# mushroonhead/spatial-intention-maps

Measured on AMD Instinct MI355X. Metric: agent-state-stacks/sec (96×96×C maps) at 1/2/4/8 MI355X; HBM GB/s vs peak, higher is better.
Workload: dtype f32

## Files before the change

spatial-intention-maps_amd/csrc/get_state_body.inc:

```
    __shared__ __attribute__((aligned(16))) char smem[LDS_BYTES];
    Shared &sh = *reinterpret_cast<Shared *>(smem);
    float *dist = reinterpret_cast<float *>(smem + OFF_DIST);
    SsspScratch &S = *reinterpret_cast<SsspScratch *>(smem + OFF_UNION);
    float *tile = reinterpret_cast<float *>(smem + OFF_UNION);

    const int n = blockIdx.x;
    const int tid = threadIdx.x;
    const int H = cfg.H, W = cfg.W;
    if (tid == 0) STAMP_NB(77);
    simaps_agent ag = agents[n];
    const int nsrc = (cfg.use_shortest_path_to_receptacle_map ? 1 : 0) + (cfg.use_shortest_path_map ? 1 : 0);
    const int cs_waves = nsrc > 0 ? 4 * nsrc : (dbg.cspace ? 4 : 0);
    const bool early_tile =
        nsrc > 0 && (cfg.room_h + 2) * sssp_pitch(cfg.room_w) * 4 <= DIST_FLOATS * 4 - CMAP_BYTES;
    uint8_t *cmap = reinterpret_cast<uint8_t *>(smem) + (early_tile ? OFF_UNION - CMAP_BYTES : OFF_CMAP);
    const bool tail_cells = early_tile && !cfg.use_distance_to_receptacle_map &&
                            tail_cells_off(cfg.room_h, cfg.room_w) + LW * LW * 2 <= DIST_FLOATS * 4;
    if (tid < 16) (&sh.bar[0][0])[tid] = 0u;
    if (tid == 16) sh.scratch_free = cs_waves == 0;
#if defined(GS_SPEC) && !GS_MIXED
    OccLoad4<512> pre8;
    OccLoad4<256> pre4;
    const bool pre_occ = (tid >> 6) < cs_waves && nsrc > 0 && occ4_ok(H, W, cfg.room_j0);
    if (pre_occ) {
        const uint8_t *occ_slot = occupancy + (size_t)ag.map_slot * H * W;
        if (cs_waves == 8) cspace_load4<512>(pre8, occ_slot, H, W, cfg.room_i0, cfg.room_j0, cfg.room_h, tid);
        else cspace_load4<256>(pre4, occ_slot, H, W, cfg.room_i0, cfg.room_j0, cfg.room_h, tid);
    }
#endif
#ifdef GS_CACHED
    char *const sc_rec = (unsigned)ag.map_slot < (unsigned)cache_records
                             ? cache + (size_t)ag.map_slot * simaps_state_cache::record_bytes(GS_ROOM_H, GS_ROOM_W)
                             : nullptr;
    CachePre sc_pre;
    if (pre_occ) cache_preload<GS_ROOM_H, GS_ROOM_W>(sc_pre, sc_rec, tid);
    bool sc_join = false;
#endif
    simaps_env ev = envs[ag.env];
    int nr_cap = SIMAPS_MAX_ROBOTS;
    if (cfg.use_intention_channels)
        nr_cap = (C - 1 - !!cfg.use_robot_map - !!cfg.use_distance_to_receptacle_map -
                  !!cfg.use_shortest_path_to_receptacle_map - !!cfg.use_shortest_path_map - !!cfg.use_history_map -
                  !!cfg.use_intention_map) / (cfg.intention_channel_spatial ? 1 : 2) + 1;
    const bool bad_desc = (unsigned)(ev.num_robots - 1) >= (unsigned)SIMAPS_MAX_ROBOTS ||
                          (unsigned)ag.robot >= (unsigned)ev.num_robots ||
                          (cfg.use_intention_channels && ev.num_robots != nr_cap);
    ev.num_robots = min(max(ev.num_robots, 1), min(nr_cap, SIMAPS_MAX_ROBOTS));
    if ((unsigned)ag.robot >= (unsigned)ev.num_robots) ag.robot = 0;
    lds_barrier();
    if (tid == 0 && bad_desc) sh.bar[0][3] = 1u;
    if (tid == 0) STAMP_NB(0);
#if GS_MIXED && defined(SIMAPS_STATE16)
    uint16_t *out = state + (size_t)out_off[n];
#elif GS_MIXED
    float *out = state + (size_t)out_off[n];
#elif defined(GS_INTO)
    auto *out = state + (size_t)into_row * LW * LW * C;
#elif defined(SIMAPS_STATE16)
    uint16_t *out = state + (size_t)n * LW * LW * C;
#else
    float *out = state + (size_t)n * LW * LW * C;
#endif
    const RenderCtx rc{cfg, sh, out, C, n};
    if ((tid >> 6) < cs_waves) {
        const Group g{tid, 64 * cs_waves, sh.bar[0], cs_waves};
#if GS_MIXED
        const uint8_t *occ_base = occupancy + ((int64_t)map_off[ag.map_slot] - (int64_t)ag.map_slot * H * W);
        if (cs_waves == 8) sweep_track<512>(sh, S, dist, cfg, geo, ag, ev, robots, occ_base, nsrc, dbg, n, g, early_tile);
        else sweep_track<256>(sh, S, dist, cfg, geo, ag, ev, robots, occ_base, nsrc, dbg, n, g, early_tile);
#elif defined(GS_CACHED)
        sc_join = sweep_track_cached<GS_ROOM_H, GS_ROOM_W>(sh, S, dist, cfg, geo, ag, ev, robots, sc_rec, pre8, sc_pre, g);
#elif defined(GS_SPEC)
        if (cs_waves == 8)
            sweep_track<512, GS_ROOM_H, GS_ROOM_W>(sh, S, dist, cfg, geo, ag, ev, robots, occupancy, nsrc, dbg, n, g,
                                                   early_tile, &pre8);
        else
            sweep_track<256, GS_ROOM_H, GS_ROOM_W>(sh, S, dist, cfg, geo, ag, ev, robots, occupancy, nsrc, dbg, n, g,
                                                   early_tile, &pre4);
#else
        if (cs_waves == 8) sweep_track<512>(sh, S, dist, cfg, geo, ag, ev, robots, occupancy, nsrc, dbg, n, g, early_tile);
        else sweep_track<256>(sh, S, dist, cfg, geo, ag, ev, robots, occupancy, nsrc, dbg, n, g, early_tile);
#endif
#ifdef GS_CACHED
        if (!sc_join) STAMP_NB(7);
    }
    if ((tid >> 6) >= cs_waves || sc_join) {
        int nw = NT / 64 - cs_waves;
        Group g{tid - 64 * cs_waves, 64 * nw, sh.bar[1], nw};
        int t = sc_join ? SC_NO_PARAM_THREAD : g.t;
#else
        STAMP_NB(7);
    } else {
        const int nw = NT / 64 - cs_waves;
        const Group g{tid - 64 * cs_waves, 64 * nw, cs_waves ? sh.bar[1] : nullptr, nw};
        const int t = g.t;
#endif
        const simaps_robot *rb = robots + ev.robot_off;
        if (t == 0) {
            sh.nr = ev.num_robots;
            sh.me = ag.robot;
            sh.env = ag.env;
            sh.has_rec = ev.has_receptacle;
        }
        if (t == 64) {
            const simaps_robot &me = rb[ag.robot];
            sh.rot = rot_params(CROP, 90.0 - me.heading * RAD_TO_DEG, cfg.rotate_rounding == SIMAPS_ROT_PLAIN);
            pos_to_pix(me.x, me.y, H, W, sh.pi, sh.pj);
            STAMP_NB(72);
        }
        if (t >= 128 && t < 128 + ev.num_robots) {
            const int k = t - 128;
            const simaps_robot &r = rb[k];
            RobotP &P = sh.rob[k];
            if ((cfg.use_intention_map && r.intention_len > SIMAPS_MAX_PATH) ||
                (cfg.use_history_map && r.history_len > SIMAPS_MAX_PATH))
                __hip_atomic_store(&sh.bar[0][3], 1u, __ATOMIC_RELAXED, __HIP_MEMORY_SCOPE_WORKGROUP);
            robot_params(P, r, cfg, geo, H, W);
            if (k == 0) STAMP_NB(73);
        }
        {
            const int w8 = t >> 6;
            const bool z8 = g.n == 512;
            const int zt = z8 ? (w8 == 3 || w8 == 4 ? t - 192 : (w8 >= 6 ? t - 256 : -1)) : t;
            const int zn = z8 ? 256 : g.n;
            if (zt >= 0) {
                uint4 *cz = reinterpret_cast<uint4 *>(cmap);
                for (int k = zt; k < CMAP_BYTES / 16; k += zn) cz[k] = uint4{0u, 0u, 0u, 0u};
                if (early_tile) {
                    uint4 *tz = reinterpret_cast<uint4 *>(tile);
                    for (int k = SCRATCH_Q + zt; k < TILE * TILE / 4; k += zn) tz[k] = uint4{0u, 0u, 0u, 0u};
                }
            }
        }
        const bool segs = (cfg.use_history_map || cfg.use_intention_map) && t >= 320 &&
                          t < 320 + ev.num_robots * SEG_PER_ROBOT;
        if (segs) {
            seg_geom(sh, cfg, rb, paths, cfg.use_history_map ? 4 : cfg.intention_map_encoding, t - 320, ag.robot);
            if (t == 320) STAMP_NB(74);
        }
        if (t < 5 * 24) sh.mwin[t] = geo.mbits[t / 24][t % 24];
        if (t >= 192 && t < 192 + 20) {
            const int q = t - 192, m = q >> 2, f = q & 3;
            sh.mwin[120 + q] = f == 0 ? geo.mrow0[m] : f == 1 ? geo.mcol0[m] : f == 2 ? geo.mnrows[m] : geo.mncols[m];
        }
        if (t == 0) STAMP_NB(75);
#ifdef GS_CACHED
        if (sc_join || cache_verdict_hit(sh)) {
            nw = 12;
            g = Group{tid - 256, 768, sh.bar[1], 12};
        }
#endif
        g.sync();
        if (t == 0) STAMP_NB(9);
        if (segs) seg_ramp(sh, t - 320);
        if (cfg.use_intention_channels && t == 256) intention_channel_order(sh, cfg, rb);
#ifdef GS_CACHED
        t = g.t;
#endif

        if (t == 0) STAMP_NB(51);
        uint32_t *cmap32 = reinterpret_cast<uint32_t *>(cmap);
        const int ci0 = sh.pi - HALF_CROP, cj0 = sh.pj - HALF_CROP;
        const int ln = t & 63, wv = __builtin_amdgcn_readfirstlane(t >> 6);
        const int nrb = ev.num_robots, wpr = nrb <= nw ? nw / nrb : 1;
        for (int kk = wv; kk < nrb * wpr; kk += nw) {
            const int k = kk % nrb, sub = kk / nrb;
            const RobotP &P = sh.rob[k];
            const int bi0 = __builtin_amdgcn_readfirstlane(P.bi0), bi1 = __builtin_amdgcn_readfirstlane(P.bi1);
            const int bj0 = P.bj0, bj1 = P.bj1, st_i = P.st_i, st_j = P.st_j;
            const int type = P.type;
            const bool cube = type == SIMAPS_LIFTING && P.lifting;
            const unsigned code0 = P.code0;
            const Rot R{P.c, P.s, P.f0, P.f1, P.S0, P.S1};
            const int *mt = reinterpret_cast<const int *>(sh.mwin + 120 + 4 * type);
            const int *mc = reinterpret_cast<const int *>(sh.mwin + 120 + 4 * 4);
            const int mt0 = mt[0], mt1 = mt[1], mt2 = mt[2], mt3 = mt[3];
            const int mc0 = mc[0], mc1 = mc[1], mc2 = mc[2], mc3 = mc[3];
            for (int rp = sub; 2 * rp <= bi1 - bi0; rp += wpr) {
                const int gi = bi0 + 2 * rp + (ln >> 5), gj = bj0 + (ln & 31);
                unsigned code = 0;
                if (gi <= bi1 && gj <= bj1) {
                    int m0, m1;
                    const bool in = rot_src(R, LW, gi - st_i, gj - st_j, m0, m1);
                    if (in) {
                        const int r = m0 - mt0, cc = m1 - mt1;
                        if ((unsigned)r < (unsigned)mt2 && (unsigned)cc < (unsigned)mt3 && ((sh.mwin[type * 24 + r] >> cc) & 1u))
                            code = code0;
                        const int r2 = m0 - mc0, c2 = m1 - mc1;
                        if (cube && (unsigned)r2 < (unsigned)mc2 && (unsigned)c2 < (unsigned)mc3 && ((sh.mwin[4 * 24 + r2] >> c2) & 1u))
                            code |= 1u << 5;
                    }
                }
                const int ca = gi - ci0, cb = gj - cj0;
                if (code && (unsigned)ca < (unsigned)CROP && (unsigned)cb < (unsigned)CROP) {
                    const int pos = ca * CROP + cb;
                    atomicOr(&cmap32[pos >> 2], code << (8 * (pos & 3)));
                }
            }
        }
#ifdef GS_SPEC
        if (early_tile && cfg.use_shortest_path_to_receptacle_map && cfg.use_shortest_path_map)
            zero_scratch_early(sh, tile, g);
#endif
        g.sync();
        if (t == 0) STAMP_NB(1);
#if GS_MIXED
        const float *ovh = overhead + (size_t)map_off[ag.map_slot];
#else
        const float *ovh = overhead + (size_t)ag.map_slot * H * W;
#endif
        if (nw == 8) render_maps<18>(rc, g, geo, ovh, rb, paths, tile, cmap, early_tile, tail_cells, dist);
        else if (nw == 12) render_maps<12>(rc, g, geo, ovh, rb, paths, tile, cmap, early_tile, tail_cells, dist);
        else render_maps<9>(rc, g, geo, ovh, rb, paths, tile, cmap, early_tile, tail_cells, dist);
        if (t == 0) STAMP_NB(8);
    }
    lds_barrier();
    STAMP(4);

    STAMP(5);
    render_distance_channels(rc, ev, dist, nsrc, reinterpret_cast<const uint16_t *>(tile),
                             tail_cells ? reinterpret_cast<const uint16_t *>(reinterpret_cast<const char *>(dist) +
                                                                          tail_cells_off(cfg.room_h, cfg.room_w))
                                        : reinterpret_cast<const uint16_t *>(tile) + LW * LW);
    STAMP(6);

    if (nsrc > 0) {
        if (dbg.sources && tid < 2) {
            int32_t *o = dbg.sources + ((size_t)n * 2 + tid) * 4;
            const int s = sh.sp_slot[tid];
            if (s >= 0) { o[0] = sh.src_q[s][0]; o[1] = sh.src_q[s][1]; o[2] = sh.src_s[s][0]; o[3] = sh.src_s[s][1]; }
            else { o[0] = o[1] = o[2] = o[3] = -1; }
        }
    }
    if (tid == 0) {
        const unsigned f = group_faults(sh.bar, sh.rounds, nsrc);
#if defined(GS_INTO) && defined(GS_INTO_KID)
        post_faults(fault, f, GS_INTO_KID, n);
#elif defined(GS_INTO)
        post_faults(fault, f, SIMAPS_K_GET_STATE_INTO, n);
#else
        post_faults(fault, f, GS_MIXED ? SIMAPS_K_GET_STATE_MIXED : SIMAPS_K_GET_STATE, n);
#endif
        if (dbg.status) {
            int st = (f & SIMAPS_FAULT_ROUNDS ? 2 : 0) | (f & SIMAPS_FAULT_TIMEOUT ? 4 : 0) |
                     (f & SIMAPS_FAULT_DESCRIPTOR ? 8 : 0);
            for (int s = 0; s < nsrc; s++) st |= sh.src_ok[s] ? 0 : 1;
            dbg.status[n] = st | ((nsrc > 0 ? sh.rounds & 0xfffff : 0) << 8);
        }
    }
#ifdef SIMAPS_PHASE_STAMPS
    if (tid == 0 && blockIdx.x < MAX_STAMP_WG) g_stamps[blockIdx.x * NSTAMP + 10] = (unsigned long long)sh.rounds;
#endif
```

spatial-intention-maps_amd/csrc/simaps_spec_cached.hip:

```cpp
#define GS_SPEC
#define GS_CACHED
#define GS_ROOM_H RH
#define GS_ROOM_W RW
#define SIMAPS_DEVICE_ONLY
#include "simaps.hip"
#include "spec.h"
#include "state_cache.h"

namespace {
using namespace simaps_state_cache;
static_assert(WIN_PAD == RMAX && WIN_ROW_U32 * 4 == (int)sizeof(uint64_t) * WIN_WORDS, "the record's window rows are SsspScratch::win's");
static_assert(sizeof(B128) == 16, "a row of free bits");

constexpr int SC_NO_PARAM_THREAD = 1 << 20;
typedef unsigned u32x4 __attribute__((ext_vector_type(4)));

__device__ __forceinline__ unsigned &sc_diff(Shared &sh) { return sh.bar[3][0]; }
__device__ __forceinline__ unsigned &sc_verdict(Shared &sh) { return sh.bar[3][3]; }

struct CachePre {
    u32x4 key[4];
    uint32_t w[OccLoad4<512>::NQ], w2;
    u32x4 pf[5];
    uint32_t pft;
};
template <int RH, int RW>
struct HitSplit {
    static constexpr int cells = (RH + 2) * ((RW + 2) | 1);
    static constexpr int ROWS = (RH + 2 + 15) / 16, FULL = cells / 4 / 256, LAST = cells / 4 - 256 * FULL, TAIL = cells & 3;
    static_assert(ROWS <= 5 && FULL == 4, "CachePre::pf holds a thread's share");
};

template <int RH, int RW>
__device__ __forceinline__ void cache_preload(CachePre &P, const char *rec, int t)
{
    const __amdgpu_buffer_rsrc_t rs =
        __builtin_amdgcn_make_buffer_rsrc((void *)rec, (short)0, rec ? record_bytes(RH, RW) : 0, 0x00020000);
    const int lane = t & 63, wave = t >> 6;
    constexpr int whM = RH + 2 * RMAX;
#pragma unroll
    for (int k = 0; k < 4; k++) P.key[k] = __builtin_amdgcn_raw_buffer_load_b128(rs, 16 * k, 0, 0);
#pragma unroll
    for (int q = 0; q < OccLoad4<512>::NQ; q++) {
        const int rr = 2 * (wave + 8 * q) + (lane >> 5);
        P.w[q] = __builtin_amdgcn_raw_buffer_load_b32(rs, rr < whM ? OFF_WIN + (rr * WIN_ROW_U32 + ((lane >> 3) & 3)) * 4 : -1, 0, 0);
    }
    const int rr = t >> 2;
    P.w2 = __builtin_amdgcn_raw_buffer_load_b32(rs, rr < whM ? OFF_WIN + (rr * WIN_ROW_U32 + 4) * 4 : -1, 0, 0);
    using HS = HitSplit<RH, RW>;
    const bool rows = wave < 4;
    const int t2 = t - 256, arr = off_rec(RH) + REC_HDR;
#pragma unroll
    for (int k = 0; k < 5; k++) {
        const int r = (t >> 4) + 16 * k;
        const int o_row = k < HS::ROWS && r >= 1 && r <= RH ? off_free(RH) + (r - 1) * 16 : -1;
        const int o_arr = k < HS::FULL || t2 < HS::LAST ? arr + (t2 + 256 * k) * 16 : -1;
        P.pf[k] = __builtin_amdgcn_raw_buffer_load_b128(rs, rows ? o_row : o_arr, 0, 0);
    }
    P.pft = __builtin_amdgcn_raw_buffer_load_b32(rs, !rows && t2 < HS::TAIL ? arr + ((HS::cells & ~3) + t2) * 4 : -1, 0, 0);
}

__device__ __forceinline__ bool win_from_dwords_cmp(SsspScratch &S, const OccLoad4<512> &L, const CachePre &P, int whM, int t)
{
    static_assert(OccLoad4<512>::NU == 1, "one tail dword per thread");
    const int lane = t & 63, wave = t >> 6;
    uint32_t *win32 = reinterpret_cast<uint32_t *>(&S.win[0][0]);
    bool diff = false;
#pragma unroll
    for (int q = 0; q < OccLoad4<512>::NQ; q++) {
        unsigned x = nib4(L.v[q]) << (4 * (lane & 7));
        x |= (unsigned)__builtin_amdgcn_mov_dpp((int)x, 0x111, 0xf, 0xf, true);
        x |= (unsigned)__builtin_amdgcn_mov_dpp((int)x, 0x112, 0xf, 0xf, true);
        x |= (unsigned)__builtin_amdgcn_mov_dpp((int)x, 0x114, 0xf, 0xf, true);
        const int rr = 2 * (wave + 8 * q) + (lane >> 5);
        if ((lane & 7) == 7 && rr < whM) {
            win32[rr * 6 + ((lane >> 3) & 3)] = x;
            diff |= x != P.w[q];
        }
    }
    {
        const int rr = t >> 2;
        unsigned x = nib4(L.v2[0]) << (4 * (t & 3));
        x |= (unsigned)__builtin_amdgcn_mov_dpp((int)x, 0x111, 0xf, 0xf, true);
        x |= (unsigned)__builtin_amdgcn_mov_dpp((int)x, 0x112, 0xf, 0xf, true);
        if ((t & 3) == 3 && rr < whM) {
            win32[rr * 6 + 4] = x;
            diff |= x != P.w2;
        }
    }
    return diff;
}

__device__ __forceinline__ bool cache_verdict_hit(Shared &sh)
{
    unsigned v = 0;
    if ((threadIdx.x & 63) == 0) {
        unsigned spins = 0;
        while (!(v = __hip_atomic_load(&sc_verdict(sh), __ATOMIC_RELAXED, __HIP_MEMORY_SCOPE_WORKGROUP))) {
            __builtin_amdgcn_s_sleep(1);
            if (++spins > (1u << 22)) {
                __hip_atomic_store(&sh.bar[1][2], 1u, __ATOMIC_RELAXED, __HIP_MEMORY_SCOPE_WORKGROUP);
                break;
            }
        }
    }
    __builtin_amdgcn_fence(__ATOMIC_ACQUIRE, "workgroup", "local");
    return (unsigned)__builtin_amdgcn_readfirstlane((int)v) == 2u;
}

template <int RH, int RW>
__device__ __forceinline__ void sssp_rounds_swapped(Shared &sh, float *dist)
{
    const int wave = __builtin_amdgcn_readfirstlane((int)threadIdx.x >> 6);
    switch ((wave + 2 * ((wave >> 2) ^ 1)) & 3) {
    case 0: sssp_rounds_word<0, RH, RW, 1>(sh, dist); break;
    case 1: sssp_rounds_word<1, RH, RW, 1>(sh, dist); break;
    case 2: sssp_rounds_word<2, RH, RW, 1>(sh, dist); break;
    default: sssp_rounds_word<3, RH, RW, 1>(sh, dist); break;
    }
}

template <int RH, int RW>
__device__ __forceinline__ bool sweep_track_cached(Shared &sh, SsspScratch &S, float *dist, const simaps_config &cfg,
                                                   const Geometry &geo, const simaps_agent &ag, const simaps_env &ev,
                                                   const simaps_robot *__restrict__ robots, char *rec,
                                                   const OccLoad4<512> &occ4, const CachePre &P, const Group &g)
{
    constexpr int h = RH, w = RW, pw = (RW + 2) | 1, cells = (h + 2) * pw, whM = h + 2 * RMAX;
    static_assert(OFF_WIN + whM * WIN_ROW_U32 * 4 <= off_free(h) && off_rec(h) + REC_HDR + cells * 4 <= record_bytes(h, w),
                  "the record's parts");
    static_assert(REC_HDR == 16 && off_rec(h) % 16 == 0 && off_free(h) % 16 == 0, "16-byte aligned parts");
    const int t = g.t, H = cfg.H, W = cfg.W;
#ifdef SIMAPS_PHASE_STAMPS
    if (t == 0 && ag.map_slot >= 0) STAMP_NB(43);
#endif
    const simaps_robot *rb = robots + ev.robot_off;
    const int radius = geo.cspace_r[rb[ag.robot].type];
    int rq0 = 0, rq1 = 0;
    if (t == 0) {
        sh.h = h;
        sh.w = w;
        sh.i0 = cfg.room_i0;
        sh.j0 = cfg.room_j0;
        pos_to_pix(ev.receptacle_x, ev.receptacle_y, H, W, rq0, rq1);
        sh.src_q[0][0] = rq0;
        sh.src_q[0][1] = rq1;
        pos_to_pix(rb[ag.robot].x, rb[ag.robot].y, H, W, sh.src_q[1][0], sh.src_q[1][1]);
        sh.sp_slot[0] = 0;
        sh.sp_slot[1] = 1;
        sh.nsrc = 2;
    }
    const u32x4 key0 = {(unsigned)SIMAPS_STATE_CACHE_MAGIC, (unsigned)H, (unsigned)W, (unsigned)cfg.room_i0};
    const u32x4 key1 = {(unsigned)cfg.room_j0, (unsigned)h, (unsigned)w, (unsigned)radius};
    const u32x4 key2 = {(unsigned)ev.has_receptacle, (unsigned)rq0, (unsigned)rq1, 0u};
    bool diff = win_from_dwords_cmp(S, occ4, P, whM, t);
    if (t == 0) {
        const u32x4 d = (P.key[0] ^ key0) | (P.key[1] ^ key1) | (P.key[2] ^ key2);
        diff |= (d.x | d.y | d.z | d.w) != 0u;
    }
    if (__ballot(diff) && (t & 63) == 0)
        __hip_atomic_fetch_or(&sc_diff(sh), 1u, __ATOMIC_RELAXED, __HIP_MEMORY_SCOPE_WORKGROUP);
    g.sync();
    if (t == 0) STAMP_NB(15);
    const bool hit = __builtin_amdgcn_readfirstlane(
                         (int)__hip_atomic_load(&sc_diff(sh), __ATOMIC_RELAXED, __HIP_MEMORY_SCOPE_WORKGROUP)) == 0;
    if (t == 0) {
#ifdef SIMAPS_DIAG_VERDICT_LATE
        for (int k = 0; k < 8; k++) __builtin_amdgcn_s_sleep(127);
#endif
        __builtin_amdgcn_fence(__ATOMIC_RELEASE, "workgroup", "local");
        __hip_atomic_store(&sc_verdict(sh), hit ? 2u : 1u, __ATOMIC_RELAXED, __HIP_MEMORY_SCOPE_WORKGROUP);
    }
    const float scale = (float)cfg.shortest_path_map_scale;
    if (hit) {
        using HS = HitSplit<RH, RW>;
        static_assert(HS::cells == cells, "the same array");
        if (t >= 256) {
            const int t2 = t - 256;
            u32x4 *d4 = reinterpret_cast<u32x4 *>(dist);
#pragma unroll
            for (int k = 0; k < HS::FULL; k++) d4[t2 + 256 * k] = P.pf[k];
            if (t2 < HS::LAST) d4[t2 + 256 * HS::FULL] = P.pf[HS::FULL];
            if (t2 < HS::TAIL) reinterpret_cast<uint32_t *>(dist)[(cells & ~3) + t2] = P.pft;
            return true;
        }
        const Group g4{t, 256, sh.bar[0], 4};
        const int qr = sh.src_q[1][0] - cfg.room_i0, qc = sh.src_q[1][1] - cfg.room_j0;
        const bool q_in = (unsigned)qr < (unsigned)h && (unsigned)qc < (unsigned)w;
        auto publish = [&](bool fr) {
            sh.src_ok[1] = fr;
            sh.src_s[1][0] = sh.src_q[1][0];
            sh.src_s[1][1] = sh.src_q[1][1];
#pragma unroll
            for (int q = 0; q < 8; q++) {
                const int d2 = (q >> 1) & 3, word = q & 1, bit = fr ? (d2 < 2 ? qr : qc) : -1;
                sh.dirty[1][d2][word] = bit >= 0 && (bit >> 6) == word ? 1ull << (bit & 63) : 0ull;
            }
        };
        const int l16 = t & 15;
        float *D1 = dist + DIST_FLOATS;
        bool own = false, own_free = false;
#pragma unroll
        for (int k = 0; k < HS::ROWS; k++) {
            const int r = (t >> 4) + 16 * k;
            if (r < h + 2) {
                const B128 f = {P.pf[k].x | ((uint64_t)P.pf[k].y << 32), P.pf[k].z | ((uint64_t)P.pf[k].w << 32)};
                if (l16 == 0 && r >= 1 && r <= h) S.freeb[r - 1] = f;
                const bool qrow = q_in && r == qr + 1;
#pragma unroll
                for (int i = 0; i < (pw + 15) / 16; i++) {
                    const int c = l16 + 16 * i;
                    if (c < pw) {
                        const bool fc = c >= 1 && c <= w && b_test(f, c - 1);
                        const bool src = qrow && c == qc + 1;
                        own |= src;
                        own_free |= src && fc;
                        D1[r * pw + c] = src && fc ? 0.0f : (fc ? INFINITY : -INFINITY);
                    }
                }
            }
        }
        if (own || (t == 0 && !q_in)) publish(own_free);
        if (t == 0) {
            const u32x4 res = P.key[3];
            sh.src_s[0][0] = (int)res.x;
            sh.src_s[0][1] = (int)res.y;
            sh.src_ok[0] = (int)res.z;
            sh.dmax[0] = __uint_as_float(res.w);
            sh.unreach[0] = (__uint_as_float(res.w) / 96.0f) * scale;
            __hip_atomic_fetch_add(reinterpret_cast<unsigned *>(rec + offsetof(simaps_state_cache_header, hits)), 1u,
                                   __ATOMIC_RELAXED, __HIP_MEMORY_SCOPE_AGENT);
        }
        if (t < 6) (&sh.changed[0][0])[t] = 0;
        if (t == 6) sh.rounds = 0;
        g4.sync();
        if (t == 0) STAMP_NB(2);
        if (!sh.src_ok[1]) {
            if (t < 64)
                snap_wave(S.freeb, h, w, cfg.room_i0, cfg.room_j0, sh.src_q[1][0], sh.src_q[1][1], [&](int si, int sj) {
                    const int sr = si - cfg.room_i0, sc = sj - cfg.room_j0;
                    if (t == 0) {
                        sh.src_s[1][0] = si;
                        sh.src_s[1][1] = sj;
                        sh.src_ok[1] = 1;
                        D1[(sr + 1) * pw + sc + 1] = 0.0f;
                    }
                    if (t < 8) {
                        const int d2 = (t >> 1) & 3, word = t & 1, bit = d2 < 2 ? sr : sc;
                        sh.dirty[1][d2][word] = (bit >> 6) == word ? 1ull << (bit & 63) : 0ull;
                    }
                });
            g4.sync();
        }
        if (t == 0) {
            STAMP_NB(48);
            __builtin_amdgcn_fence(__ATOMIC_RELEASE, "workgroup", "local");
            __hip_atomic_store(&sh.scratch_free, 1, __ATOMIC_RELAXED, __HIP_MEMORY_SCOPE_WORKGROUP);
            STAMP_NB(3);
        }
        sssp_rounds_swapped<RH, RW>(sh, dist);
        const float m = max_finite_part(D1, cells, t, 256);
        if ((t & 63) == 0) sh.red[1][t >> 6] = m;
        g4.sync();
        if (t == 0) STAMP_NB(49);
        if (t == 1) {
            float mm = sh.red[1][0];
            for (int k = 1; k < 4; k++) mm = fmaxf(mm, sh.red[1][k]);
            sh.dmax[1] = mm;
            sh.unreach[1] = (mm / 96.0f) * scale;
        }
        if (t == 0) STAMP_NB(50);
        return false;
    }
    build_cspace<512>(S, nullptr, h, w, radius, g, dist, 2, &occ4, nullptr, H, W, cfg.room_i0, cfg.room_j0, true);
    if (t == 0) STAMP_NB(2);
    if (rec) {
        const uint32_t *win32 = reinterpret_cast<const uint32_t *>(&S.win[0][0]);
        uint32_t *rw = reinterpret_cast<uint32_t *>(rec + OFF_WIN);
        for (int k = t; k < whM * WIN_ROW_U32; k += 512)
            if (k % WIN_ROW_U32 != 5) rw[k] = win32[k];
        if (t < h) reinterpret_cast<B128 *>(rec + off_free(h))[t] = S.freeb[t];
    }
    snap_init_sources(sh, S, dist, 2, g);
    if (t == 0) {
        STAMP_NB(48);
        __builtin_amdgcn_fence(__ATOMIC_RELEASE, "workgroup", "local");
        __hip_atomic_store(&sh.scratch_free, 1, __ATOMIC_RELAXED, __HIP_MEMORY_SCOPE_WORKGROUP);
        STAMP_NB(3);
    }
    sssp_rounds_swapped<RH, RW>(sh, dist);
    {
        const int s = (t >> 8) ^ 1;
        if (rec && s == 0) rec_export(rec + off_rec(h), dist, h, w, sh.src_ok[0], nullptr, t & 255, 256);
        const float m = max_finite_part(dist + s * DIST_FLOATS, cells, t & 255, 256);
        if ((t & 63) == 0) sh.red[s][(t >> 6) & 3] = m;
    }
    g.sync();
    if (t == 0) STAMP_NB(49);
    sssp_max_final(sh, 2, 4, scale, t);
    if (rec && t == 0) {
        const bool good = sh.rounds < (1 << 20);
        u32x4 *hd = reinterpret_cast<u32x4 *>(rec);
        hd[0] = u32x4{good ? key0[0] : 0u, key0[1], key0[2], key0[3]};
        hd[1] = key1;
        hd[2] = key2;
        const bool ok0 = sh.src_ok[0] != 0;
        hd[3] = u32x4{ok0 ? (unsigned)sh.src_s[0][0] : ~0u, ok0 ? (unsigned)sh.src_s[0][1] : ~0u, ok0 ? 1u : 0u,
                      __float_as_uint(sh.dmax[0])};
        __hip_atomic_fetch_add(reinterpret_cast<unsigned *>(rec + offsetof(simaps_state_cache_header, misses)), 1u,
                               __ATOMIC_RELAXED, __HIP_MEMORY_SCOPE_AGENT);
    }
    if (t == 0) STAMP_NB(50);
    return false;
}

template <int MH, int MW, int RH, int RW>
__global__ void __launch_bounds__(NT) get_state_cached_kernel(
    simaps_config cfg_in, Geometry geo, const simaps_agent *__restrict__ agents, const simaps_env *__restrict__ envs,
    const simaps_robot *__restrict__ robots, const double *__restrict__ paths, const uint8_t *__restrict__ occupancy,
    const float *__restrict__ overhead, float *__restrict__ state, int C, unsigned *fault, char *cache, int cache_records)
{
    simaps_config cfg = cfg_in;
    cfg.use_robot_map = 1;
    cfg.use_distance_to_receptacle_map = 0;
    cfg.use_shortest_path_to_receptacle_map = 1;
    cfg.use_shortest_path_map = 1;
    cfg.use_intention_map = 1;
    cfg.use_history_map = 0;
    cfg.use_intention_channels = 0;
    cfg.layout_chw = 1;
    cfg.H = MH;
    cfg.W = MW;
    cfg.room_h = RH;
    cfg.room_w = RW;
    const simaps_debug dbg = {};
#define GS_MIXED 0
#include "get_state_body.inc"
#undef GS_MIXED
}
}

namespace simaps_state_cache {
void launch_get_state(const simaps_config &cfg, const simaps::Geometry &geo, int N, const simaps_agent *agents,
                      const simaps_env *envs, const simaps_robot *robots, const double *paths,
                      const uint8_t *occupancy, const float *overhead, float *state, int C, unsigned *fault,
                      void *cache, int cache_records, hipStream_t stream)
{
    constexpr int MH = SIMAPS_ROOM_SMALL_H, MW = SIMAPS_ROOM_SMALL_W, RH = SIMAPS_ROOM_SMALL_RH, RW = SIMAPS_ROOM_SMALL_RW;
    hipLaunchKernelGGL((get_state_cached_kernel<MH, MW, RH, RW>), dim3(N), dim3(NT), 0, stream, cfg, geo, agents, envs,
                       robots, paths, occupancy, overhead, state, C, fault, (char *)cache, cache_records);
}

#if defined(SIMAPS_PHASE_STAMPS) || defined(SIMAPS_LIGHT_STAMPS)
int read_stamps(unsigned long long *host_out)
{
    return hipMemcpyFromSymbol(host_out, HIP_SYMBOL(g_stamps), sizeof(g_stamps)) == hipSuccess ? 0 : SIMAPS_EHIP;
}
#endif
}
```

Baseline: 10.98 million.

## Load cached distance array straight into LDS with buffer-load DMA on hit

On a cache hit, the cached distance array is no longer preloaded into registers by the upper waves and then stored to LDS. It is fetched after the verdict using buffer_load ... lds, which writes directly into shared memory, and the wait is deferred until just before the map-rendering group sync. Preload loads are also restricted to the waves that use them (key only in wave 0, window rows only for in-range waves), which lowers register pressure and wasted VMEM issue. The trade-off is that the array fetch now starts only after the hit verdict rather than being prefetched, so its latency has to be hidden behind the cmap/render work. It also relies on hand-written inline asm that manipulates M0.

```diff
diff --git a/spatial-intention-maps_amd/csrc/get_state_body.inc b/spatial-intention-maps_amd/csrc/get_state_body.inc
--- a/spatial-intention-maps_amd/csrc/get_state_body.inc
+++ b/spatial-intention-maps_amd/csrc/get_state_body.inc
@@ -202,6 +202,9 @@
         if (early_tile && cfg.use_shortest_path_to_receptacle_map && cfg.use_shortest_path_map)
             zero_scratch_early(sh, tile, g);
 #endif
+#if defined(GS_CACHED) && !defined(SIMAPS_DIAG_ARRAY_LATE)
+        if (sc_join) sc_retire_array();
+#endif
         g.sync();
         if (t == 0) STAMP_NB(1);
 #if GS_MIXED
@@ -214,6 +217,12 @@
         else render_maps<9>(rc, g, geo, ovh, rb, paths, tile, cmap, early_tile, tail_cells, dist);
         if (t == 0) STAMP_NB(8);
     }
+#if defined(GS_CACHED) && defined(SIMAPS_DIAG_ARRAY_LATE)
+    if (sc_join) {
+        hit_array_dma<GS_ROOM_H, GS_ROOM_W>(dist, sc_rec, tid - 256);
+        sc_retire_array();
+    }
+#endif
     lds_barrier();
     STAMP(4);
 
diff --git a/spatial-intention-maps_amd/csrc/simaps_spec_cached.hip b/spatial-intention-maps_amd/csrc/simaps_spec_cached.hip
--- a/spatial-intention-maps_amd/csrc/simaps_spec_cached.hip
+++ b/spatial-intention-maps_amd/csrc/simaps_spec_cached.hip
@@ -21,44 +21,100 @@
 struct CachePre {
     u32x4 key[4];
     uint32_t w[OccLoad4<512>::NQ], w2;
-    u32x4 pf[5];
-    uint32_t pft;
+    u32x4 pf[3];
 };
 template <int RH, int RW>
 struct HitSplit {
     static constexpr int cells = (RH + 2) * ((RW + 2) | 1);
-    static constexpr int ROWS = (RH + 2 + 15) / 16, FULL = cells / 4 / 256, LAST = cells / 4 - 256 * FULL, TAIL = cells & 3;
-    static_assert(ROWS <= 5 && FULL == 4, "CachePre::pf holds a thread's share");
+    static constexpr int ROWS = (RH + 2 + 15) / 16, PIECES = cells * 4 / 1024, REST = cells - 256 * PIECES;
+    static_assert(ROWS <= 3 && REST >= 0 && REST <= 64, "CachePre::pf holds a thread's rows; one wave-instruction for the rest");
 };
 
 template <int RH, int RW>
+struct RecordRsrc {
+    static constexpr unsigned FLAGS = 0x00020000u;
+    __device__ static __forceinline__ int len(const char *rec) { return rec ? record_bytes(RH, RW) : 0; }
+    __device__ static __forceinline__ __amdgpu_buffer_rsrc_t builtin(const char *rec)
+    {
+        return __builtin_amdgcn_make_buffer_rsrc((void *)rec, (short)0, len(rec), (int)FLAGS);
+    }
+    __device__ static __forceinline__ u32x4 words(const char *rec)
+    {
+        auto u = [](unsigned x) { return (unsigned)__builtin_amdgcn_readfirstlane((int)x); };
+        const uint64_t base = (uint64_t)(uintptr_t)rec;
+        return u32x4{u((unsigned)base), u((unsigned)(base >> 32) & 0xffffu), u((unsigned)len(rec)), FLAGS};
+    }
+};
+
+template <int RH, int RW>
 __device__ __forceinline__ void cache_preload(CachePre &P, const char *rec, int t)
 {
-    const __amdgpu_buffer_rsrc_t rs =
-        __builtin_amdgcn_make_buffer_rsrc((void *)rec, (short)0, rec ? record_bytes(RH, RW) : 0, 0x00020000);
-    const int lane = t & 63, wave = t >> 6;
+    const __amdgpu_buffer_rsrc_t rs = RecordRsrc<RH, RW>::builtin(rec);
+    const int lane = t & 63, wave = __builtin_amdgcn_readfirstlane(t >> 6);
     constexpr int whM = RH + 2 * RMAX;
-#pragma unroll
-    for (int k = 0; k < 4; k++) P.key[k] = __builtin_amdgcn_raw_buffer_load_b128(rs, 16 * k, 0, 0);
+    static_assert(whM % 2 == 0, "a wave's two window rows are in or out together");
+#pragma unroll
+    for (int k = 0; k < 4; k++) {
+        P.key[k] = u32x4{0u, 0u, 0u, 0u};
+        if (wave == 0) P.key[k] = __builtin_amdgcn_raw_buffer_load_b128(rs, 16 * k, 0, 0);
+    }
 #pragma unroll
     for (int q = 0; q < OccLoad4<512>::NQ; q++) {
         const int rr = 2 * (wave + 8 * q) + (lane >> 5);
-        P.w[q] = __builtin_amdgcn_raw_buffer_load_b32(rs, rr < whM ? OFF_WIN + (rr * WIN_ROW_U32 + ((lane >> 3) & 3)) * 4 : -1, 0, 0);
+        P.w[q] = 0u;
+        if (2 * (wave + 8 * q) < whM)
+            P.w[q] = __builtin_amdgcn_raw_buffer_load_b32(rs, OFF_WIN + (rr * WIN_ROW_U32 + ((lane >> 3) & 3)) * 4, 0, 0);
     }
     const int rr = t >> 2;
-    P.w2 = __builtin_amdgcn_raw_buffer_load_b32(rs, rr < whM ? OFF_WIN + (rr * WIN_ROW_U32 + 4) * 4 : -1, 0, 0);
+    P.w2 = 0u;
+    if (16 * wave < whM)
+        P.w2 = __builtin_amdgcn_raw_buffer_load_b32(rs, rr < whM ? OFF_WIN + (rr * WIN_ROW_U32 + 4) * 4 : -1, 0, 0);
     using HS = HitSplit<RH, RW>;
-    const bool rows = wave < 4;
-    const int t2 = t - 256, arr = off_rec(RH) + REC_HDR;
-#pragma unroll
-    for (int k = 0; k < 5; k++) {
+#pragma unroll
+    for (int k = 0; k < HS::ROWS; k++) {
         const int r = (t >> 4) + 16 * k;
-        const int o_row = k < HS::ROWS && r >= 1 && r <= RH ? off_free(RH) + (r - 1) * 16 : -1;
-        const int o_arr = k < HS::FULL || t2 < HS::LAST ? arr + (t2 + 256 * k) * 16 : -1;
-        P.pf[k] = __builtin_amdgcn_raw_buffer_load_b128(rs, rows ? o_row : o_arr, 0, 0);
-    }
-    P.pft = __builtin_amdgcn_raw_buffer_load_b32(rs, !rows && t2 < HS::TAIL ? arr + ((HS::cells & ~3) + t2) * 4 : -1, 0, 0);
-}
+        P.pf[k] = u32x4{0u, 0u, 0u, 0u};
+        if (wave < 4) P.pf[k] = __builtin_amdgcn_raw_buffer_load_b128(rs, r >= 1 && r <= RH ? off_free(RH) + (r - 1) * 16 : -1, 0, 0);
+    }
+}
+
+template <int BYTES>
+__device__ __forceinline__ void sc_dma_piece(u32x4 rs, unsigned lds_base, int voffset)
+{
+    static_assert(BYTES == 16 || BYTES == 4, "");
+    unsigned keep;
+    if (BYTES == 16)
+        asm volatile("s_mov_b32 %0, m0\n\ts_mov_b32 m0, %3\n\ts_nop 0\n\tbuffer_load_dwordx4 %1, %2, 0 offen lds\n\ts_mov_b32 m0, %0"
+                     : "=&s"(keep)
+                     : "v"(voffset), "s"(rs), "s"(lds_base)
+                     : "memory");
+    else
+        asm volatile("s_mov_b32 %0, m0\n\ts_mov_b32 m0, %3\n\ts_nop 0\n\tbuffer_load_dword %1, %2, 0 offen lds\n\ts_mov_b32 m0, %0"
+                     : "=&s"(keep)
+                     : "v"(voffset), "s"(rs), "s"(lds_base)
+                     : "memory");
+}
+template <int RH, int RW>
+__device__ __forceinline__ void hit_array_dma(float *dist, const char *rec, int t2)
+{
+    using HS = HitSplit<RH, RW>;
+    constexpr int arr = off_rec(RH) + REC_HDR;
+    static_assert(arr % 16 == 0 && OFF_DIST % 16 == 0, "16-byte pieces");
+    static_assert(arr + 1024 * HS::PIECES + 4 * HS::REST == arr + 4 * HS::cells && arr + 4 * HS::cells <= record_bytes(RH, RW),
+                  "the DMA covers the array and stays inside the record");
+    auto u = [](unsigned x) { return (unsigned)__builtin_amdgcn_readfirstlane((int)x); };
+    const u32x4 rs = RecordRsrc<RH, RW>::words(rec);
+    const int lane = t2 & 63, wave = __builtin_amdgcn_readfirstlane(t2 >> 6);
+    const unsigned d = u((unsigned)(uintptr_t)(__attribute__((address_space(3))) char *)reinterpret_cast<char *>(dist));
+#pragma unroll
+    for (int k = 0; k < (HS::PIECES + 3) / 4; k++) {
+        const int p = wave + 4 * k;
+        if (p < HS::PIECES) sc_dma_piece<16>(rs, d + 1024 * p, arr + 1024 * p + 16 * lane);
+    }
+    if (HS::REST > 0 && wave == (HS::PIECES & 3) && lane < HS::REST)
+        sc_dma_piece<4>(rs, d + 1024 * HS::PIECES, arr + 1024 * HS::PIECES + 4 * lane);
+}
+__device__ __forceinline__ void sc_retire_array() { asm volatile("s_waitcnt vmcnt(0)" ::: "memory"); }
 
 __device__ __forceinline__ bool win_from_dwords_cmp(SsspScratch &S, const OccLoad4<512> &L, const CachePre &P, int whM, int t)
 {
@@ -176,12 +232,9 @@
         using HS = HitSplit<RH, RW>;
         static_assert(HS::cells == cells, "the same array");
         if (t >= 256) {
-            const int t2 = t - 256;
-            u32x4 *d4 = reinterpret_cast<u32x4 *>(dist);
-#pragma unroll
-            for (int k = 0; k < HS::FULL; k++) d4[t2 + 256 * k] = P.pf[k];
-            if (t2 < HS::LAST) d4[t2 + 256 * HS::FULL] = P.pf[HS::FULL];
-            if (t2 < HS::TAIL) reinterpret_cast<uint32_t *>(dist)[(cells & ~3) + t2] = P.pft;
+#ifndef SIMAPS_DIAG_ARRAY_LATE
+            hit_array_dma<RH, RW>(dist, rec, t - 256);
+#endif
             return true;
         }
         const Group g4{t, 256, sh.bar[0], 4};
```

Result: faster. 11.28 million (median of 6 runs) (+2.8%).
